# ShawnHymel/ei-keyword-spotting

Hardware: AMD Instinct MI355X
Metric: 1s@16kHz clips/sec (MFCC+CNN) (higher is better)
Workload: dtype f32

## Files before the change

ei-keyword-spotting_amd/csrc/kws_api.cpp:

```cpp
#include "kws_internal.h"

#pragma GCC visibility push(default)
extern "C" {

EI_IMPULSE_ERROR kws_create(const void *blob, size_t nbytes, int device, kws_handle **out)
{
    if (!blob || !out) return fail(KWS_ERROR_BAD_ARGUMENT, "null argument");
    *out = nullptr;
    kws_handle *h = new kws_handle();
    h->device = device;
    if (!parse_model(blob, nbytes, h->model)) { delete h; return fail(KWS_ERROR_BAD_ARGUMENT, "not a valid .kwsm model blob"); }
    int ndev = 0;
    if (hipGetDeviceCount(&ndev) != hipSuccess || ndev <= 0) {
        delete h;
        return fail(KWS_ERROR_HIP, "no HIP device available (libkws_mi355x has no CPU fallback)");
    }
    if (device < 0 || device >= ndev) { delete h; return fail(KWS_ERROR_HIP, "device %d out of range (%d devices)", device, ndev); }
    if (hipSetDevice(device) != hipSuccess) { delete h; return fail(KWS_ERROR_HIP, "hipSetDevice(%d) failed", device); }
    hipDeviceProp_t prop;
    if (hipGetDeviceProperties(&prop, device) == hipSuccess) h->n_cu = prop.multiProcessorCount;
    EI_IMPULSE_ERROR e = build_dsp_plan(h);
    if (e == EI_IMPULSE_OK) e = build_nn_plan(h);
    if (e == EI_IMPULSE_OK) e = build_fast_plans(h);
    if (e != EI_IMPULSE_OK) { kws_destroy(h); return e; }
// ... 13 lines not shown
    while ((n = fread(tmp, 1, sizeof(tmp), f)) > 0) buf.insert(buf.end(), tmp, tmp + n);
    fclose(f);
    return kws_create(buf.data(), buf.size(), device, out);
}

void kws_destroy(kws_handle *h)
{
    if (!h) return;
    kws_sdk_forget_default(h);
    (void)hipSetDevice(h->device);
    if (h->scratch_ev) { (void)hipEventSynchronize(h->scratch_ev); (void)hipEventDestroy(h->scratch_ev); }
    for (void *p : h->dev_allocs) (void)hipFree(p);
    if (h->s_mfcc) (void)hipFree(h->s_mfcc);
    if (h->s_q) (void)hipFree(h->s_q);
    if (h->d_flags) (void)hipFree(h->d_flags);
    if (h->d_flags2) (void)hipFree(h->d_flags2);
    if (h->d_flags3) (void)hipFree(h->d_flags3);
    if (h->s_cep) (void)hipFree(h->s_cep);
    if (h->scan_release) h->scan_release(h);
    for (hipEvent_t ev : h->gen_tune.ev) if (ev) (void)hipEventDestroy(ev);
    for (auto &g : h->g_sets) for (void *p : { (void *)g.ws, (void *)g.mfcc, (void *)g.feat }) if (p) (void)hipFree(p);
    for (int k = 0; k < 2; ++k) {
        for (void *p : { (void *)h->pipe.pcm[k], (void *)h->pipe.s[k], (void *)h->pipe.f[k], (void *)h->pipe.q[k] }) if (p) (void)hipFree(p);
        if (h->pipe.st[k]) (void)hipStreamDestroy(h->pipe.st[k]);
    }
    for (void *p : { (void *)h->ws.d_x, (void *)h->ws.d_f, (void *)h->ws.d_s, (void *)h->ws.d_w, (void *)h->ws.d_q })
        if (p) (void)hipFree(p);
    for (void *p : { (void *)h->ws.h_x, (void *)h->ws.h_s, (void *)h->ws.h_f })
        if (p) (void)hipHostFree(p);
    for (hipEvent_t ev : h->ws.ev) if (ev) (void)hipEventDestroy(ev);
// ... 123 lines not shown
    *count = 0;
    std::lock_guard<std::mutex> lk(h->mu);
    if (!h->d_flags2) return EI_IMPULSE_OK;
    HIP_TRY(hipSetDevice(h->device));
    HIP_TRY(hipDeviceSynchronize());
    int n = 0;
    HIP_TRY(hipMemcpy(&n, h->d_flags2, sizeof(int), hipMemcpyDeviceToHost));
    *count = (size_t)n;
    return EI_IMPULSE_OK;
}

static EI_IMPULSE_ERROR ensure_flags(kws_handle *h, size_t B)
{
    if (B + 1 <= h->flags_cap) return EI_IMPULSE_OK;
    if (h->d_flags) (void)hipFree(h->d_flags);
    if (h->d_flags2) (void)hipFree(h->d_flags2);
    if (h->d_flags3) (void)hipFree(h->d_flags3);
    h->d_flags = h->d_flags2 = h->d_flags3 = nullptr; h->flags_cap = 0;
    HIP_TRY(hipMalloc((void **)&h->d_flags, (B + 1) * sizeof(int)));
    HIP_TRY(hipMalloc((void **)&h->d_flags2, (B + 1) * sizeof(int)));
    HIP_TRY(hipMalloc((void **)&h->d_flags3, (B + 1) * sizeof(int)));
    HIP_TRY(hipMemset(h->d_flags2, 0, sizeof(int)));
    h->flags_cap = B + 1;
    return EI_IMPULSE_OK;
}

static EI_IMPULSE_ERROR classify_fast_device(kws_handle *h, const int16_t *pcm, size_t B, float *scores, float *fx, bool want_f, int8_t *q,
                                             hipStream_t s);
static EI_IMPULSE_ERROR classify_device(kws_handle *h, const int16_t *pcm, size_t B, float *scores, float *f, int8_t *q, hipStream_t s);
int grid_cap_mfcc(const kws_handle *h) { return h->n_cu * 8; }
int grid_cap_nn(const kws_handle *h) { return h->n_cu * 4; }

static const size_t kGenTuneMinClips = 2048;
static int generic_chunk_begin(kws_handle *h, size_t B, hipStream_t s, bool *mine)
{
    *mine = false;
    const char *fe = KWS_DEV_ENV("KWS_DEV_GENERIC_LCH");
// ... 414 lines not shown
    if (rc) return fail(KWS_ERROR_HIP, "quantise kernel launch failed: %s", hipGetErrorString((hipError_t)rc));
    return kws_nn_batch_device(h, h->s_q, B, scores, nullptr, nullptr, nullptr, stream);
}

static EI_IMPULSE_ERROR rerun_flagged_device(kws_handle *h, const int16_t *pcm, size_t B, float *scores, float *fx, bool want_f, int8_t *q, hipStream_t s)
{
    static const bool skip = KWS_DEV_ENV("KWS_DEV_FAST_NO_RERUN") != nullptr;
    if (skip) return EI_IMPULSE_OK;
    const size_t F = h->model.nn_input_frame_size;
    if (B > h->cep_cap) {
        if (h->s_cep) (void)hipFree(h->s_cep);
        h->s_cep = nullptr; h->cep_cap = 0;
        HIP_TRY(hipMalloc((void **)&h->s_cep, B * F * sizeof(float)));
        h->cep_cap = B;
    }
    HIP_TRY(hipMemsetAsync(h->d_flags2, 0, sizeof(int), s));
    int rc = kws_launch_spectral(h->dsp, pcm, 0, (int)B, h->s_cep, nullptr, 0, grid_cap_mfcc(h), s, h->d_flags);
    if (rc) return fail(KWS_ERROR_HIP, "MFCC kernel launch failed: %s", hipGetErrorString((hipError_t)rc));
    const bool fused = scores && h->is_float && h->fast_fused_ok;
    if (!scores || (fused && want_f) || !fused) {
        rc = kws_launch_fast_from_cepstra(h->dsp, h->fast_plain, h->d_fast_plain, h->s_cep, (int)B, nullptr, (h->is_float || want_f) ? fx : nullptr, q,
                                          h->nn.in_scale, h->nn.in_zp, h->d_flags2, h->d_flags2 + 1, h->n_cu, s, h->d_flags);
        if (rc) return fail(KWS_ERROR_HIP, "fast kernel launch failed: %s", hipGetErrorString((hipError_t)rc));
        if (fused) HIP_TRY(hipMemsetAsync(h->d_flags3, 0, sizeof(int), s));
    }
    if (fused) {
        int *const fl = want_f ? h->d_flags3 : h->d_flags2;
        rc = kws_launch_fast_from_cepstra(h->dsp, h->fast_fused_cep, h->d_fast_fused_cep, h->s_cep, (int)B, scores, nullptr, nullptr, h->nn.in_scale, h->nn.in_zp,
                                          fl, fl + 1, h->n_cu, s, h->d_flags, h->tap_logits);
        if (rc) return fail(KWS_ERROR_HIP, "fast kernel launch failed: %s", hipGetErrorString((hipError_t)rc));
    } else if (scores) {
// ... 7 lines not shown
    if (rc) return fail(KWS_ERROR_HIP, "CMVN kernel launch failed: %s", hipGetErrorString((hipError_t)rc));
    if (!scores) return EI_IMPULSE_OK;
    if (h->is_float) rc = kws_launch_nn_f32(h->nnf, h->d_nnf, fx, (int)B, scores, h->tap_logits, h->n_cu, s, h->d_flags2);
    else if (!ran_nn) rc = kws_launch_nn(h->nn, q, (int)B, scores, nullptr, h->pooled_tap_bytes, nullptr, nullptr, grid_cap_nn(h), s, h->d_flags2);
    if (rc) return fail(KWS_ERROR_HIP, "NN kernel launch failed: %s", hipGetErrorString((hipError_t)rc));
    return EI_IMPULSE_OK;
}

static EI_IMPULSE_ERROR classify_fast_device(kws_handle *h, const int16_t *pcm, size_t B, float *scores, float *fx, bool want_f, int8_t *q,
                                             hipStream_t s)
{
    if (B > 0x7fffffff) return fail(KWS_ERROR_BAD_ARGUMENT, "batch too large");
    if (((uintptr_t)pcm & 15) != 0) return fail(KWS_ERROR_BAD_ARGUMENT, "pcm must be 16-byte aligned");
    EI_IMPULSE_ERROR e = ensure_flags(h, B);
    if (e) return e;
    HIP_TRY(hipMemsetAsync(h->d_flags, 0, sizeof(int), s));
    const bool fused = scores && h->is_float && h->fast_fused_ok;
    int rc = 0;
    if (h->model.dsp.block == DSP_BLOCK_MFE) {
        const KwsDspPlan &P = h->dsp;
        const int rows = P.n_frames, cols = P.n_filters;
        if (rows > (cols > 16 ? 51 : 52) || P.win_size < (cols > 16 ? 17 : 13))
            return fail(KWS_ERROR_UNSUPPORTED_MODEL, "%d frames x %d filters, window %d outside the MFE normalisation kernel's limits", rows, cols, P.win_size);
        rc = kws_launch_fast(P, h->fast_plain, h->d_fast_plain, pcm, (int)B, nullptr, fx, nullptr, h->nn.in_scale, h->nn.in_zp, h->d_flags, h->d_flags + 1, h->n_cu, s);
        if (rc) return fail(KWS_ERROR_HIP, "fast kernel launch failed: %s (is the gfx950 code object present?)", hipGetErrorString((hipError_t)rc));
        rc = kws_launch_mfe_norm(fx, (int)B, rows, cols, P.win_size, P.pad_map, rows + 2 * P.pad, grid_cap_nn(h), s);
        if (!rc && q) rc = kws_launch_quantize(fx, q, B * h->model.nn_input_frame_size, h->nn.in_scale, h->nn.in_zp, s);
        if (rc) return fail(KWS_ERROR_HIP, "MFE block launch failed: %s", hipGetErrorString((hipError_t)rc));
        if (!scores) return EI_IMPULSE_OK;
        if (h->is_float) return nn_f32_device(h, fx, B, scores, h->tap_logits, s);
        rc = kws_launch_nn(h->nn, q, (int)B, scores, nullptr, h->pooled_tap_bytes, nullptr, nullptr, grid_cap_nn(h), s);
        if (rc) return fail(KWS_ERROR_HIP, "NN kernel launch failed: %s", hipGetErrorString((hipError_t)rc));
        return EI_IMPULSE_OK;
// ... 14 lines not shown
        if (h->fast_entry_tier >= 3) {
            HIP_TRY(hipMemsetAsync(h->d_flags2, 0, sizeof(int), s));
            if (!scores) return mfcc_fused_device(h, pcm, 0, B, fx, q, s);
            return classify_device(h, pcm, B, scores, fx, q, s);
        }
        const size_t F = h->model.nn_input_frame_size;
        if (B > h->cep_cap) {
            if (h->s_cep) (void)hipFree(h->s_cep);
            h->s_cep = nullptr; h->cep_cap = 0;
            HIP_TRY(hipMalloc((void **)&h->s_cep, B * F * sizeof(float)));
            h->cep_cap = B;
        }
        if ((e = spectral_device(h, h->dsp, pcm, 0, B, h->s_cep, nullptr, s))) return e;
        return cmvn_nn_fast_device(h, h->s_cep, B, scores, s, 0, 0, want_f ? fx : nullptr, q);
    }
    if (scores && !h->is_float && h->fast_q_ok) {
        rc = kws_launch_fast(h->dsp, h->fast_q, h->d_fast_q, pcm, (int)B, scores, want_f ? fx : nullptr, q != h->s_q ? q : nullptr, h->nn.in_scale, h->nn.in_zp,
                             h->d_flags, h->d_flags + 1, h->n_cu, s, h->d_nn);
        if (rc) return fail(KWS_ERROR_HIP, "fast kernel launch failed: %s (is the gfx950 code object present?)", hipGetErrorString((hipError_t)rc));
        return rerun_flagged_device(h, pcm, B, scores, fx, want_f, q, s);
    }
#ifdef KWS_DEV_SWITCHES
    if (fused && KWS_DEV_ENV("KWS_DEV_FAST_SPLIT")) {
        rc = kws_launch_fast(h->dsp, h->fast_plain, h->d_fast_plain, pcm, (int)B, nullptr, fx, nullptr, h->nn.in_scale, h->nn.in_zp, h->d_flags, h->d_flags + 1, h->n_cu, s);
        if (rc) return fail(KWS_ERROR_HIP, "fast kernel launch failed: %s", hipGetErrorString((hipError_t)rc));
        HIP_TRY(hipMemsetAsync(h->d_flags3, 0, sizeof(int), s));
        rc = kws_launch_fast_from_cepstra(h->dsp, h->fast_fused_cep, h->d_fast_fused_cep, fx, (int)B, scores, nullptr, nullptr, h->nn.in_scale, h->nn.in_zp,
                                          h->d_flags3, h->d_flags3 + 1, h->n_cu, s, nullptr, h->tap_logits, 1);
        if (rc) return fail(KWS_ERROR_HIP, "fast kernel launch failed: %s", hipGetErrorString((hipError_t)rc));
        return EI_IMPULSE_OK;
    }
#endif
    if (fused && want_f) {
        rc = kws_launch_fast(h->dsp, h->fast_plain, h->d_fast_plain, pcm, (int)B, nullptr, fx, nullptr, h->nn.in_scale, h->nn.in_zp, h->d_flags, h->d_flags + 1,
                             h->n_cu, s);
        if (rc) return fail(KWS_ERROR_HIP, "fast kernel launch failed: %s (is the gfx950 code object present?)", hipGetErrorString((hipError_t)rc));
        HIP_TRY(hipMemsetAsync(h->d_flags3, 0, sizeof(int), s));
    }
    const KwsFastPlan &FP = fused ? h->fast_fused : h->fast_plain;
    int *const fl = (fused && want_f) ? h->d_flags3 : h->d_flags;
    rc = kws_launch_fast(h->dsp, FP, fused ? h->d_fast_fused : h->d_fast_plain, pcm, (int)B, scores, fused ? nullptr : fx, fused ? nullptr : q, h->nn.in_scale,
                         h->nn.in_zp, fl, fl + 1, h->n_cu, s, nullptr, h->tap_logits);
    if (rc) return fail(KWS_ERROR_HIP, "fast kernel launch failed: %s (is the gfx950 code object present?)", hipGetErrorString((hipError_t)rc));
    if (scores && !fused) {
        if (h->is_float) { if ((e = nn_f32_device(h, fx, B, scores, h->tap_logits, s))) return e; }
        else {
            rc = kws_launch_nn(h->nn, q, (int)B, scores, nullptr, h->pooled_tap_bytes, nullptr, nullptr, grid_cap_nn(h), s);
            if (rc) return fail(KWS_ERROR_HIP, "NN kernel launch failed: %s", hipGetErrorString((hipError_t)rc));
        }
    }
    return rerun_flagged_device(h, pcm, B, scores, fx, want_f, q, s);
}

static EI_IMPULSE_ERROR classify_device(kws_handle *h, const int16_t *pcm, size_t B, float *scores, float *f, int8_t *q, hipStream_t s)
{
    EI_IMPULSE_ERROR e;
    if (h->is_float) {
        e = mfcc_fused_device(h, pcm, 0, B, f, nullptr, s);
// ... 139 lines not shown
```

ei-keyword-spotting_amd/csrc/kws_fast.h:

```cpp
#pragma once
#include <stdint.h>

#include "kws_plan.h"

#define KWS_FAST_MAX_BLOCKS 8
#define KWS_FAST_NZ_MAX 12
#define KWS_FAST_NZ2 8
#define KWS_FAST_DCT_GROUPS 5
#define KWS_FAST_MEL_CHUNK 8
#define KWS_FAST_CMVN_EXT 8
#define KWS_FAST_XS 144
#define KWS_FAST_WAVE 64
#ifndef KWS_FAST_WPS
#define KWS_FAST_WPS 2
#endif
#define KWS_FAST_ZF 320

struct KwsFastBlock {
    int in_w, in_c, in_cp;
    int out_c, taps, pad_left, out_w;
    int pool, pool_stride, pool_w;
    int in_stride;
    int m_tiles, n_tiles;
    int vrows;
// ... 43 lines not shown
    int fs, f_floats, r1_floats, wave_floats, shared_floats, n_waves;
    int zero_off;
    int sink_off;
    int stash_off;
    const float *shared_init;
    int qnet, q_floats;
    int mfe;
    int fuse, n_blocks;
    KwsFastBlock blk[KWS_FAST_MAX_BLOCKS];
    int fc_in, fc_out, fc_w_off, fc_b_off;
    float fc_min, fc_max, beta;
    int n_labels;
    int wps;
    int twl_off;
    int *tickets;
};
```

ei-keyword-spotting_amd/csrc/kws_fast.hip:

```cpp
#include <atomic>

#include "kws_device.h"
#include "kws_fast.h"
#if KWS_FAST_WPS >= 3
#define kws_fast_kernel kws_fast_kernel_w3
#define kws_launch_fast kws_launch_fast_w3
#define kws_launch_fast_prof kws_launch_fast_prof_w3
#endif
#include "kws_nn_int8_dev.h"

typedef float v4f __attribute__((ext_vector_type(4)));
#if KWS_FAST_WPS >= 3
#define KWS_OPAQUE3(v) asm volatile("" : "+v"(v))
#define KWS_FAST_SINK (shared + FP.sink_off)
#else
#define KWS_OPAQUE3(v) do { } while (0)
#define KWS_FAST_SINK (F + FP.sink_off)
#endif
static_assert(KWS_FAST_ZF == KWS_ZF && KWS_FAST_WAVE == KWS_WAVE, "kws_fast.h mirrors kws_device.h");

template <int CTRL> __device__ __forceinline__ float dpp_mov(float v)
{
    return __int_as_float(__builtin_amdgcn_update_dpp(0, __float_as_int(v), CTRL, 0xf, 0xf, true));
}
// ... 770 lines not shown
    }
    WAVE_SYNC();
    return vacc;
}

#define KWS_FAST_NPHASE 20
#define FPH(i) do { if (PROF) { const long long now_ = clock64(); ph[i] += now_ - tlast; tlast = now_; } } while (0)

template <int NZ, int DG, bool PROF = false, bool FROM_CEP = false, bool NET = true, int QCP = 0, bool MFE = false>
__global__ __launch_bounds__(256 * KWS_FAST_WPS, KWS_FAST_WPS) void kws_fast_kernel(KwsDspPlan P, const KwsFastPlan *__restrict__ FPp, const int16_t *__restrict__ pcm, int n_clips,
                                                          float *__restrict__ scores, float *__restrict__ features,
                                                          int8_t *__restrict__ q_out, float in_scale, int in_zp,
                                                          int *__restrict__ flag_count, int *__restrict__ flag_list,
                                                          long long *__restrict__ prof_out = nullptr, const float *__restrict__ cep = nullptr,
                                                          const KwsNnPlan *__restrict__ QNp = nullptr, const int *__restrict__ sel = nullptr,
                                                          float *__restrict__ tap_logits = nullptr, int feat_in = 0)
{
    static_assert(QCP == 0 || !NET, "the int8 network follows the feature-emitting form");
    static_assert(!MFE || (!NET && QCP == 0 && !FROM_CEP && !PROF), "the MFE form is the spectral prefix: mel energies to HBM");
    const KwsFastPlan &FP = *FPp;
    extern __shared__ __attribute__((aligned(16))) float lds[];
    const int lane = threadIdx.x & (KWS_WAVE - 1), wave = __builtin_amdgcn_readfirstlane((int)(threadIdx.x >> 6));
    if (FROM_CEP && (int)blockIdx.x * (int)(blockDim.x >> 6) >= sel_count(sel, n_clips)) return;
    float *shared = lds;
    float *F = lds + FP.shared_floats + FP.q_floats + wave * FP.wave_floats;
    float *R1 = F + FP.f_floats;
    float *xw = R1, *pw = R1;
    for (int i = threadIdx.x; i < FP.shared_floats; i += blockDim.x) shared[i] = FP.shared_init[i];
    for (int i = lane; i < FP.r1_floats; i += KWS_WAVE) R1[i] = 0.0f;
    constexpr int Q_HEAD = 48 * 256, Q_WB1 = Q_HEAD + ((KWS_HEAD_BYTES + 15) & ~15), Q_WB2 = Q_WB1 + (QCP == 16 ? 4 : 16) * KWS_WAVE * 16,
                  Q_RQ = Q_WB2 + 4 * KWS_WAVE * 16;
    if constexpr (QCP != 0) {
        unsigned char *const qs = (unsigned char *)(lds + FP.shared_floats);
        const KwsNnPlan &QN = *QNp;
        for (int i = threadIdx.x * 4; i < QN.blk[0].out_c * 256; i += blockDim.x * 4) *(int *)(qs + i) = *(const int *)(QN.blk[0].add_lut + i);
        for (int i = threadIdx.x * 4; i < QN.blk[1].out_c * 256; i += blockDim.x * 4) *(int *)(qs + 32 * 256 + i) = *(const int *)(QN.blk[1].add_lut + i);
// ... 397 lines not shown
                    prow[0] = pdc;
                }
                esum = half_wave_sum(esum);
                if (t == 0 && live_t) *((pair_tail && half == 1) ? stash + 47 : elog + ft) = fast_log(esum == 0.0f ? FLT_EPSILON : esum);
            }
            mel_phase(KWS_FAST_MEL_CHUNK * n_pass, pair_tail ? 2 : n_tail, 1, pair_tail ? (int)(stash - img) - nfr * fs : 0);
            have_stash = pair_tail;
            WAVE_SYNC();
        }

        if constexpr (!MFE) {
            int lane_l = lane;
            asm volatile("" : "+v"(lane_l));
            const int lm = lane_l & 15, lq = lane_l >> 4;
            float dB[DG][2][2];
#pragma unroll
            for (int g = 0; g < DG; ++g)
#pragma unroll
                for (int i = 0; i < 2; ++i)
#pragma unroll
                    for (int nt = 0; nt < 2; ++nt) dB[g][i][nt] = dct_frag[((g * 2 + i) * 2 + nt) * KWS_WAVE + lane_l];
            const float *arow = img + lm * fs + 2 * lq;
            float e0 = 0.0f;
            if (lane_l < nfr) e0 = elog[lane_l];
            v4f acc[4][2];
            __builtin_amdgcn_s_setprio(1);
#pragma unroll
            for (int rnd = 0; rnd < 2; ++rnd) {
                float2 a[2][DG];
#pragma unroll
                for (int m2 = 0; m2 < 2; ++m2)
#pragma unroll
                    for (int g = 0; g < DG; ++g) a[m2][g] = *(const float2 *)(arow + 16 * (2 * rnd + m2) * fs + 8 * g);
#pragma unroll
                for (int m2 = 0; m2 < 2; ++m2) { acc[2 * rnd + m2][0] = v4f{ 0.f, 0.f, 0.f, 0.f }; acc[2 * rnd + m2][1] = v4f{ 0.f, 0.f, 0.f, 0.f }; }
#pragma unroll
// ... 260 lines not shown
    if (lane == 0) {
        const int gone = __hip_atomic_fetch_add(FP.tickets + 1, 1, __ATOMIC_RELAXED, __HIP_MEMORY_SCOPE_AGENT);
        if (gone == (int)(gridDim.x * (blockDim.x >> 6)) - 1) {
            __hip_atomic_store(FP.tickets, 0, __ATOMIC_RELAXED, __HIP_MEMORY_SCOPE_AGENT);
            __hip_atomic_store(FP.tickets + 1, 0, __ATOMIC_RELAXED, __HIP_MEMORY_SCOPE_AGENT);
        }
    }
#endif
    if (PROF && blockIdx.x == 0 && threadIdx.x == 0 && prof_out)
        for (int i = 0; i < KWS_FAST_NPHASE; ++i) prof_out[i] = ph[i];
}

#ifndef KWS_FAST_NO_LAUNCHERS
#if KWS_FAST_WPS < 3
int kws_launch_fast_w3(const KwsDspPlan &P, const KwsFastPlan &FP, const KwsFastPlan *d_plan, const int16_t *pcm, int n_clips, float *scores, float *features,
                       int8_t *q_out, float in_scale, int in_zp, int *flag_count, int *flag_list, int n_cu, hipStream_t stream, const KwsNnPlan *d_nn, float *tap_logits);
int kws_launch_fast_prof_w3(const KwsDspPlan &P, const KwsFastPlan &FP, const KwsFastPlan *d_plan, const int16_t *pcm, int n_clips, float *scores,
                            int *flag_count, int *flag_list, int n_cu, long long *prof_out, hipStream_t stream);
#endif
template <int NZ, int DG, bool PROF, bool FROM_CEP = false, bool NET = true, int QCP = 0, bool MFE = false>
static int launch_fast_t(const KwsDspPlan &P, const KwsFastPlan &FP, const KwsFastPlan *d_plan, const int16_t *pcm, int n_clips, float *scores,
                         float *features, int8_t *q_out, float in_scale, int in_zp, int *flag_count, int *flag_list, int n_cu,
                         long long *prof_out, hipStream_t stream, const float *cep = nullptr, const KwsNnPlan *d_nn = nullptr, const int *sel = nullptr,
                         float *tap_logits = nullptr, int feat_in = 0)
{
    const size_t smem = ((size_t)FP.shared_floats + FP.q_floats + (size_t)FP.n_waves * FP.wave_floats) * sizeof(float);
    static std::atomic<unsigned long long> attr_done{ 0 };
    int dev = 0;
    if (hipGetDevice(&dev) != hipSuccess) return (int)hipGetLastError();
    const unsigned long long bit = 1ull << (dev & 63);
    if (!(attr_done.load(std::memory_order_acquire) & bit)) {
        if (hipFuncSetAttribute((const void *)kws_fast_kernel<NZ, DG, PROF, FROM_CEP, NET, QCP, MFE>, hipFuncAttributeMaxDynamicSharedMemorySize, 160 * 1024) != hipSuccess)
            return (int)hipGetLastError();
        attr_done.fetch_or(bit, std::memory_order_release);
    }
    const int per_wg = FP.n_waves;
    int grid = (n_clips + per_wg - 1) / per_wg;
    if (grid > n_cu) grid = n_cu;
#if KWS_FAST_WPS >= 3
    if (!FP.tickets) return (int)hipErrorInvalidValue;
#endif
    hipLaunchKernelGGL((kws_fast_kernel<NZ, DG, PROF, FROM_CEP, NET, QCP, MFE>), dim3(grid), dim3(KWS_WAVE * FP.n_waves), smem, stream, P, d_plan, pcm, n_clips, scores,
                       features, q_out, in_scale, in_zp, flag_count, flag_list, prof_out, cep, d_nn, sel, tap_logits, feat_in);
    return (int)hipGetLastError();
}

int kws_launch_fast(const KwsDspPlan &P, const KwsFastPlan &FP, const KwsFastPlan *d_plan, const int16_t *pcm, int n_clips, float *scores,
                    float *features, int8_t *q_out, float in_scale, int in_zp, int *flag_count, int *flag_list, int n_cu, hipStream_t stream,
                    const KwsNnPlan *d_nn, float *tap_logits)
{
    (void)hipGetLastError();
    if (n_clips <= 0) return 0;
#define KWS_FAST_ARGS P, FP, d_plan, pcm, n_clips, scores, features, q_out, in_scale, in_zp, flag_count, flag_list, n_cu, nullptr, stream
#define KWS_FAST_NARGS KWS_FAST_ARGS, nullptr, nullptr, nullptr, tap_logits
#if KWS_FAST_WPS >= 3
    if (FP.wps != KWS_FAST_WPS || FP.qnet || FP.mfe || !FP.fuse) return (int)hipErrorInvalidValue;
#define KWS_FAST_PLAIN(...) ((int)hipErrorInvalidValue)
#else
#define KWS_FAST_PLAIN(...) (__VA_ARGS__)
    if (FP.wps >= 3) return kws_launch_fast_w3(P, FP, d_plan, pcm, n_clips, scores, features, q_out, in_scale, in_zp, flag_count, flag_list, n_cu, stream, d_nn, tap_logits);
    if (FP.qnet) {
#define KWS_FAST_QARGS P, FP, d_plan, pcm, n_clips, scores, features, q_out, in_scale, in_zp, flag_count, flag_list, n_cu, nullptr, stream, nullptr, d_nn
        if (FP.qnet == 16 && FP.dct_groups == 4)
            return FP.nz <= 4 ? launch_fast_t<4, 4, false, false, false, 16>(KWS_FAST_QARGS) : FP.nz <= 8 ? launch_fast_t<8, 4, false, false, false, 16>(KWS_FAST_QARGS)
                                                                                                          : launch_fast_t<KWS_FAST_NZ_MAX, 4, false, false, false, 16>(KWS_FAST_QARGS);
        if (FP.qnet == 64 && FP.dct_groups == 5)
            return FP.nz <= 4 ? launch_fast_t<4, 5, false, false, false, 64>(KWS_FAST_QARGS) : FP.nz <= 8 ? launch_fast_t<8, 5, false, false, false, 64>(KWS_FAST_QARGS)
                                                                                                          : launch_fast_t<KWS_FAST_NZ_MAX, 5, false, false, false, 64>(KWS_FAST_QARGS);
        return (int)hipErrorInvalidValue;
    }
    if (FP.mfe) {
        if (scores || q_out || !features) return (int)hipErrorInvalidValue;
        if (FP.dct_groups == 4)
            return FP.nz <= 4 ? launch_fast_t<4, 4, false, false, false, 0, true>(KWS_FAST_ARGS) : FP.nz <= 8 ? launch_fast_t<8, 4, false, false, false, 0, true>(KWS_FAST_ARGS)
                                                                                                            : launch_fast_t<KWS_FAST_NZ_MAX, 4, false, false, false, 0, true>(KWS_FAST_ARGS);
        if (FP.dct_groups == 5)
            return FP.nz <= 4 ? launch_fast_t<4, 5, false, false, false, 0, true>(KWS_FAST_ARGS) : FP.nz <= 8 ? launch_fast_t<8, 5, false, false, false, 0, true>(KWS_FAST_ARGS)
// ... 58 lines not shown
```

ei-keyword-spotting_amd/csrc/kws_fast_plan.cpp:

```cpp
#include "kws_internal.h"
#include <atomic>
#include <cstdlib>

static const int kLdsBytes = 160 * 1024;

static int round_up(int v, int m) { return (v + m - 1) / m * m; }

static uint16_t f32_to_f16(float f)
{
    uint32_t u;
    memcpy(&u, &f, sizeof u);
    const uint32_t sign = (u >> 16) & 0x8000u;
    u &= 0x7fffffffu;
    if (u >= 0x47800000u) return (uint16_t)(sign | (u > 0x7f800000u ? 0x7e00u : 0x7c00u));
    if (u < 0x38800000u) {
        if (u < 0x33000000u) return (uint16_t)sign;
        const int shift = 126 - (int)(u >> 23);
        const uint32_t m = (u & 0x7fffffu) | 0x800000u;
        uint32_t h = m >> shift;
        const uint32_t rem = m & ((1u << shift) - 1u), half = 1u << (shift - 1);
        if (rem > half || (rem == half && (h & 1u))) h++;
        return (uint16_t)(sign | h);
    }
    uint32_t h = ((u - 0x38000000u) >> 13);
// ... 140 lines not shown
        F.c0_abs = scale * kFloorCep * per_dev;
        F.c0_rel = scale * std::min(kappa, kappa_0) * per_dev;
        F.c0_inv_rows = 1.0f / (float)nfr;
    }
    F.sys_t2 = (h->is_float && h->gain.calibrated) ? kSysRatio * kSysRatio : 0.0f;
    F.pad_off = (int)shared.size();
    for (int v : pmap) { float f; memcpy(&f, &v, sizeof f); shared.push_back(f); }
    F.sil_off = -1;
    if ((int)h->fast_sil_row.size() == ncep && !KWS_DEV_ENV("KWS_DEV_FAST_NO_SILENT_ROW")) {
        while (shared.size() & 3) shared.push_back(0.0f);
        F.sil_off = (int)shared.size();
        for (int c = 0; c < 32; c++) shared.push_back((c >= 1 && c <= NF / 2 && c < ncep) ? h->fast_sil_row[(size_t)c] : 0.0f);
    }
}

static EI_IMPULSE_ERROR build_fast_dsp(kws_handle *h, KwsFastPlan &F, std::vector<float> &shared)
{
    const Model &m = h->model;
    const DspCfg &c = m.dsp;
    const KwsDspPlan &P = h->dsp;
    const int NF = c.num_filters, nfr = P.n_frames, ncep = P.n_cepstral;
    F.mfe = c.block == DSP_BLOCK_MFE ? 1 : 0;
    if (P.generic) return fail(KWS_ERROR_UNSUPPORTED_MODEL, "fast mode serves the configurations of the tuned MFCC kernel (fft 256, 32 / 40 filters, "
                                                            "up to 52 aligned frames); this model runs on the general kernels");
    if (c.fft_length != 256) return fail(KWS_ERROR_UNSUPPORTED_MODEL, "fast mode: fft_length %d (kernel is built for 256)", c.fft_length);
    if (NF != 32 && NF != 40) return fail(KWS_ERROR_UNSUPPORTED_MODEL, "fast mode: %d mel filters (the kernel is instantiated for 32 and 40)", NF);
    if ((ncep <= 16 || F.wps >= 3) && nfr <= 52) { F.cr = 13; F.cg = 16; }
    else if (nfr <= 51) { F.cr = 17; F.cg = 20; }
    else return fail(KWS_ERROR_UNSUPPORTED_MODEL, "fast mode: %d frames x %d cepstra outside the cmvnw layouts", nfr, ncep);
    if (nfr < 2) return fail(KWS_ERROR_UNSUPPORTED_MODEL, "fast mode: %d frames", nfr);

// ... 114 lines not shown
        h_twiddles(c.fft_length / 2, tw);
        h_super_twiddles(c.fft_length / 2, stw);
        while (shared.size() & 3) shared.push_back(0.0f);
        F.twl_off = (int)shared.size();
        for (int fl = 0; fl < 8; fl++)
            for (int a = 0; a < 4; a++)
                for (int m = 1; m <= 3; m++) { const float2 v = tw[(size_t)m * (fl + 8 * a)]; shared.push_back(v.x); shared.push_back(v.y); }
        for (int fl = 0; fl < 8; fl++)
            for (int q = 0; q < 8; q++) {
                const int k = fl + 8 * (q & 3) + 32 * (q >> 2);
                const float2 v = stw[(size_t)(k == 0 ? c.fft_length / 4 : k) - 1];
                shared.push_back(v.x); shared.push_back(v.y);
            }
    }
    while (shared.size() & 3) shared.push_back(0.0f);
    F.dct_off = (int)shared.size();
    shared.insert(shared.end(), frag.begin(), frag.end());
    return EI_IMPULSE_OK;
}

static void fast_wave_floats(const kws_handle *h, KwsFastPlan &F, int need_f, int need_r1)
{
    const int nfr = h->dsp.n_frames;
    if (F.wps >= 3) {
        F.f_floats = round_up(std::max(nfr * F.fs + nfr, need_f), 4) + 48;
    } else {
        F.f_floats = round_up(std::max(nfr * F.fs + nfr, need_f), 4) + KWS_FAST_WAVE + 48;
        F.sink_off = F.f_floats - KWS_FAST_WAVE - 48;
    }
    F.stash_off = F.f_floats - 48;
// ... 75 lines not shown
    std::vector<float> shared;
    EI_IMPULSE_ERROR e = build_fast_dsp(h, F, shared);
    if (e) return e;
    F.fs = h->dsp.n_filters + 4;
    F.fuse = 0;
    F.n_labels = (int)h->model.labels.size();
    F.qnet = qcp;
    F.q_floats = (int)((kws_fast_qnet_bytes(qcp) + 15) / 16 * 4);
    if (!h->d_nn) {
        std::vector<KwsNnPlan> one(1, h->nn);
        if ((e = h->upload(one, &h->d_nn))) return e;
    }
    return finish_fast_plan(h, F, shared, 24 * 8 + 96, 72 * qcp / 4);
}

static EI_IMPULSE_ERROR build_fast_fused(kws_handle *h, int wps, KwsFastPlan &F)
{
    memset(&F, 0, sizeof(F));
    F.wps = wps;
    if (!h->is_float) return fail(KWS_ERROR_UNSUPPORTED_MODEL, "fast mode: the fused network is float32 (int8 graphs keep their exact kernels)");
    if (h->fast_plain.mfe) return fail(KWS_ERROR_UNSUPPORTED_MODEL, "fast mode: the MFE block's normalisation sits between the front end and the network (not fused)");
    const KwsNnPlanF32 &N = h->nnf;
    if (N.n_blocks > KWS_FAST_MAX_BLOCKS) return fail(KWS_ERROR_UNSUPPORTED_MODEL, "fast mode: %d conv blocks", N.n_blocks);
    if (N.fc_out > KWS_FAST_WAVE) return fail(KWS_ERROR_UNSUPPORTED_MODEL, "fast mode: %d outputs", N.fc_out);
    std::vector<float> shared;
    EI_IMPULSE_ERROR e = build_fast_dsp(h, F, shared);
    if (e) return e;
    F.fuse = 1;
    F.n_blocks = N.n_blocks;
    F.n_labels = N.n_labels;
    F.fs = h->dsp.n_filters + 4;
    int need[2] = { 0, 0 };
    std::vector<uint16_t> hfrag[KWS_FAST_MAX_BLOCKS];
    const bool hconv_on = !KWS_DEV_ENV("KWS_DEV_FAST_F32_CONV");
    while (shared.size() & 3) shared.push_back(0.0f);
    F.zero_off = (int)shared.size();
    shared.resize(shared.size() + 64, 0.0f);
    for (int b = 0; b < N.n_blocks; b++) {
        const KwsConvBlockF32 &s = N.blk[b];
        KwsFastBlock &k = F.blk[b];
        k.dw = s.depthwise ? 1 : 0; k.mult = s.depth_mult;
        k.in_w = s.in_w; k.in_c = s.in_c; k.in_cp = round_up(s.in_c, 8);
        k.out_c = s.out_c; k.taps = s.taps; k.pad_left = s.pad_left; k.out_w = s.out_w;
        k.pool = s.pool; k.pool_stride = s.pool_stride; k.pool_w = s.pool_w;
        k.in_stride = b == 0 ? F.fs : k.in_cp + 4;
        k.m_tiles = (s.out_w + 15) / 16; k.n_tiles = (s.out_c + 15) / 16;
// ... 115 lines not shown
        k.dw_seg_rows = (k.out_w + k.dw_nseg - 1) / k.dw_nseg;
    }
    return finish_fast_plan(h, F, shared, need[0], need[1]);
}

EI_IMPULSE_ERROR build_fast_plans(kws_handle *h)
{
    if (h->is_float && !h->dsp.generic && h->nnf.n_blocks > 0 && h->nnf.blk[0].in_w == h->dsp.n_frames && h->nnf.blk[0].in_c == h->dsp.n_cepstral)
        kws_calibrate_gain(h);
    record_silent_row(h);
    h->fast_plain_ok = build_fast_plain(h) == EI_IMPULSE_OK;
    if (!h->fast_plain_ok) h->fast_why = kws_last_error();
    int want_wps = h->fast_entry_tier <= 1 ? 3 : 2, min_waves3 = 11;
    if (const char *ev = KWS_DEV_ENV("KWS_DEV_FAST_WPS")) { want_wps = atoi(ev) >= 3 ? 3 : 2; min_waves3 = 4; }
    h->fast_fused_ok = h->fast_plain_ok && build_fast_fused(h, want_wps, h->fast_fused) == EI_IMPULSE_OK;
    if (h->fast_plain_ok && want_wps >= 3 && (!h->fast_fused_ok || h->fast_fused.n_waves < min_waves3))
        h->fast_fused_ok = build_fast_fused(h, 2, h->fast_fused) == EI_IMPULSE_OK;
    if (h->fast_fused_ok) {
        if (h->fast_fused.wps >= 3) h->fast_fused_ok = build_fast_fused(h, 2, h->fast_fused_cep) == EI_IMPULSE_OK;
        else { h->fast_fused_cep = h->fast_fused; h->d_fast_fused_cep = h->d_fast_fused; }
    }
    if (h->fast_plain_ok && !h->fast_fused_ok) h->fast_why = kws_last_error();
    h->fast_q_ok = h->fast_plain_ok && !h->is_float && build_fast_q(h) == EI_IMPULSE_OK;
    if (h->fast_plain_ok && !h->is_float && !h->fast_q_ok) h->fast_why = kws_last_error();
    return EI_IMPULSE_OK;
}
```

ei-keyword-spotting_amd/csrc/kws_internal.h:

```cpp
#pragma once
#include <hip/hip_runtime.h>

#include <float.h>
#include <math.h>
#include <stdarg.h>
#include <stdio.h>
#include <stdlib.h>
#include <string.h>
#include <time.h>

#include <mutex>
#include <string>
#include <map>
#include <vector>

#include "../../include/kws/kws.h"
#include "kws_plan.h"
#include "kws_fast.h"

int kws_launch_spectral(const KwsDspPlan &P, const void *pcm, int pcm_is_float, int n_clips, float *mfcc_out, const float *wrap,
                        int out_stride, int grid_cap, hipStream_t stream, const int *sel = nullptr);
int kws_launch_maf(float *scores, float *running_sum, float *maf_buf, int n, int buf_idx, int taps, hipStream_t stream);
int kws_launch_unring(const float *src, float *dst, int n_streams, int rows, int cols, int ring_rows, int head, hipStream_t stream);
int kws_launch_mfe(const KwsDspPlan &P, const void *pcm, int pcm_is_float, int n_clips, float *mel_out, float *energy_out, const float *wrap,
// ... 5 lines not shown
                               int in_zp, int grid_cap, long long *prof_out, hipStream_t stream);
int kws_launch_cmvn_nn(const KwsDspPlan &P, const KwsNnPlan &N, const float *mfcc, int n_clips, float *features, int8_t *q_out,
                       float *scores, int8_t *tap_pooled, int pooled_stride, int8_t *tap_fc, int8_t *tap_out_q, int grid_cap,
                       int *ran_nn, hipStream_t stream, const int *sel = nullptr);
int kws_launch_fast_from_cepstra(const KwsDspPlan &P, const KwsFastPlan &FP, const KwsFastPlan *d_plan, const float *cep, int n_clips, float *scores,
                                 float *features, int8_t *q_out, float in_scale, int in_zp, int *flag_count, int *flag_list, int n_cu, hipStream_t stream,
                                 const int *sel = nullptr, float *tap_logits = nullptr, int feat_in = 0);
int kws_launch_nn_f32(const KwsNnPlanF32 &N, const KwsNnPlanF32 *d_plan, const float *features, int n_clips, float *scores,
                      float *tap_logits, int n_cu, hipStream_t stream, const int *sel = nullptr);
size_t kws_nn_f32_smem_bytes(const KwsNnPlanF32 &N, int n_waves);
void kws_nn_f32_pick_blocking(KwsConvBlockF32 *k);
int kws_launch_nn(const KwsNnPlan &N, const int8_t *q_in, int n_clips, float *scores, int8_t *tap_pooled,
                  int pooled_stride, int8_t *tap_fc, int8_t *tap_out_q, int grid_cap, hipStream_t stream, const int *sel = nullptr);
int kws_launch_fast(const KwsDspPlan &P, const KwsFastPlan &FP, const KwsFastPlan *d_plan, const int16_t *pcm, int n_clips, float *scores, float *features,
                    int8_t *q_out, float in_scale, int in_zp, int *flag_count, int *flag_list, int n_cu, hipStream_t stream, const KwsNnPlan *d_nn = nullptr,
                    float *tap_logits = nullptr);
size_t kws_fast_qnet_bytes(int qcp);
int kws_launch_fast_prof(const KwsDspPlan &P, const KwsFastPlan &FP, const KwsFastPlan *d_plan, const int16_t *pcm, int n_clips, float *scores,
                         int *flag_count, int *flag_list, int n_cu, long long *prof_out, hipStream_t stream);
int kws_launch_mix_audio(const float *words, const int *word_len, size_t word_stride, const float *noise, const int *start, float word_vol,
                         float bg_vol, int n, size_t n_clips, int16_t *out, hipStream_t stream);
int kws_launch_quantize(const float *f, int8_t *q, size_t n, float scale, int zp, hipStream_t stream);
int kws_launch_resample(const float *in, size_t n_in, float *out, size_t n_out, size_t n_valid, double ratio, const double *win, const double *delta, int nwin,
                        int precision, int exact, const double *treg, hipStream_t stream);
size_t kws_generic_ws_bytes(const KwsDspPlan &P, int grid);
bool kws_generic_uses_lds(const KwsDspPlan &P);
int kws_launch_spectral_generic(const KwsDspPlan &P, const void *pcm, int pcm_is_float, int n_clips, float *mfcc_out, const float *wrap,
                                int out_stride, float *ws, int grid, int lch , hipStream_t stream);
int kws_launch_cmvn_generic(const KwsDspPlan &P, const float *mfcc, int n_clips, float *features, int8_t *q_out, float in_scale, int in_zp,
                            hipStream_t stream);
int kws_launch_synth(uint32_t seed, uint32_t first_clip, uint32_t n_clips, uint32_t clip_len, int16_t *out, hipStream_t stream);
// ... 133 lines not shown
    struct Gain { std::vector<float> col; float sigma_net = 0.0f, total = 0.0f; int calibrated = 0, n_inputs = 0; } gain;
    KwsFastPlan fast_plain{}, fast_fused{}, fast_q{};
    const KwsFastPlan *d_fast_plain = nullptr, *d_fast_fused = nullptr, *d_fast_q = nullptr;
    KwsFastPlan fast_fused_cep{};
    const KwsFastPlan *d_fast_fused_cep = nullptr;
    const KwsNnPlan *d_nn = nullptr;
    bool fast_plain_ok = false, fast_fused_ok = false, fast_q_ok = false;
    std::string fast_why;
    std::vector<float> fast_guard_coef[2][4];
    int fast_dev_overrides = 0;
    int fast_entry_tier = 1;
    std::vector<float> fast_sil_row;
    std::vector<float> fast_gain_used;
    int mode = KWS_MODE_EXACT;
    int *d_flags = nullptr;
    int *d_flags2 = nullptr;
    int *d_flags3 = nullptr;
    float *tap_logits = nullptr;
    float *s_cep = nullptr;
    struct KwsScanScratch *scan = nullptr;
    void (*scan_release)(kws_handle *) = nullptr;
    size_t flags_cap = 0, cep_cap = 0;

    template <typename T> EI_IMPULSE_ERROR upload(const std::vector<T> &v, const T **out)
    {
        void *d = nullptr;
        size_t nb = std::max<size_t>(v.size() * sizeof(T), 16);
        HIP_TRY(hipMalloc(&d, nb));
        dev_allocs.push_back(d);
        if (!v.empty()) HIP_TRY(hipMemcpy(d, v.data(), v.size() * sizeof(T), hipMemcpyHostToDevice));
// ... 72 lines not shown
```

Before: 52.70 million.

## Zero flag counters inside fast kernel via double-buffered flags instead of memsets

Removes the per-call hipMemsetAsync launches for the flag counters. It double-buffers d_flags so the fast kernel's first thread clears the next call's counter and the rerun counter. It also adds an opt-in compact fused plan that keeps the DCT fragment in global memory instead of LDS, which can raise the wave count. The compact path is gated behind a dev env switch. The ping-pong scheme assumes the counter for the next call is consumed before the kernel that zeroes it runs.

```diff
diff --git a/ei-keyword-spotting_amd/csrc/kws_api.cpp b/ei-keyword-spotting_amd/csrc/kws_api.cpp
--- a/ei-keyword-spotting_amd/csrc/kws_api.cpp
+++ b/ei-keyword-spotting_amd/csrc/kws_api.cpp
@@ -51,6 +51,7 @@
     if (h->s_mfcc) (void)hipFree(h->s_mfcc);
     if (h->s_q) (void)hipFree(h->s_q);
     if (h->d_flags) (void)hipFree(h->d_flags);
+    if (h->d_flags_alt) (void)hipFree(h->d_flags_alt);
     if (h->d_flags2) (void)hipFree(h->d_flags2);
     if (h->d_flags3) (void)hipFree(h->d_flags3);
     if (h->s_cep) (void)hipFree(h->s_cep);
@@ -204,13 +205,16 @@
 {
     if (B + 1 <= h->flags_cap) return EI_IMPULSE_OK;
     if (h->d_flags) (void)hipFree(h->d_flags);
+    if (h->d_flags_alt) (void)hipFree(h->d_flags_alt);
     if (h->d_flags2) (void)hipFree(h->d_flags2);
     if (h->d_flags3) (void)hipFree(h->d_flags3);
-    h->d_flags = h->d_flags2 = h->d_flags3 = nullptr; h->flags_cap = 0;
+    h->d_flags = h->d_flags_alt = h->d_flags2 = h->d_flags3 = nullptr; h->flags_cap = 0;
     HIP_TRY(hipMalloc((void **)&h->d_flags, (B + 1) * sizeof(int)));
+    HIP_TRY(hipMalloc((void **)&h->d_flags_alt, (B + 1) * sizeof(int)));
     HIP_TRY(hipMalloc((void **)&h->d_flags2, (B + 1) * sizeof(int)));
     HIP_TRY(hipMalloc((void **)&h->d_flags3, (B + 1) * sizeof(int)));
     HIP_TRY(hipMemset(h->d_flags2, 0, sizeof(int)));
+    HIP_TRY(hipMemset(h->d_flags_alt, 0, sizeof(int)));
     h->flags_cap = B + 1;
     return EI_IMPULSE_OK;
 }
@@ -655,7 +659,6 @@
         HIP_TRY(hipMalloc((void **)&h->s_cep, B * F * sizeof(float)));
         h->cep_cap = B;
     }
-    HIP_TRY(hipMemsetAsync(h->d_flags2, 0, sizeof(int), s));
     int rc = kws_launch_spectral(h->dsp, pcm, 0, (int)B, h->s_cep, nullptr, 0, grid_cap_mfcc(h), s, h->d_flags);
     if (rc) return fail(KWS_ERROR_HIP, "MFCC kernel launch failed: %s", hipGetErrorString((hipError_t)rc));
     const bool fused = scores && h->is_float && h->fast_fused_ok;
@@ -693,9 +696,9 @@
     if (((uintptr_t)pcm & 15) != 0) return fail(KWS_ERROR_BAD_ARGUMENT, "pcm must be 16-byte aligned");
     EI_IMPULSE_ERROR e = ensure_flags(h, B);
     if (e) return e;
-    HIP_TRY(hipMemsetAsync(h->d_flags, 0, sizeof(int), s));
     const bool fused = scores && h->is_float && h->fast_fused_ok;
     int rc = 0;
+    if (h->model.dsp.block == DSP_BLOCK_MFE || (h->fast_entry_tier >= 2 && (scores || want_f || q))) HIP_TRY(hipMemsetAsync(h->d_flags, 0, sizeof(int), s));
     if (h->model.dsp.block == DSP_BLOCK_MFE) {
         const KwsDspPlan &P = h->dsp;
         const int rows = P.n_frames, cols = P.n_filters;
@@ -740,16 +743,20 @@
         if ((e = spectral_device(h, h->dsp, pcm, 0, B, h->s_cep, nullptr, s))) return e;
         return cmvn_nn_fast_device(h, h->s_cep, B, scores, s, 0, 0, want_f ? fx : nullptr, q);
     }
+    std::swap(h->d_flags, h->d_flags_alt);
+    int *const zero_a = h->d_flags_alt, *const zero_b = h->d_flags2;
+    auto first_launch_failed = [h]() { std::swap(h->d_flags, h->d_flags_alt); };
     if (scores && !h->is_float && h->fast_q_ok) {
         rc = kws_launch_fast(h->dsp, h->fast_q, h->d_fast_q, pcm, (int)B, scores, want_f ? fx : nullptr, q != h->s_q ? q : nullptr, h->nn.in_scale, h->nn.in_zp,
-                             h->d_flags, h->d_flags + 1, h->n_cu, s, h->d_nn);
-        if (rc) return fail(KWS_ERROR_HIP, "fast kernel launch failed: %s (is the gfx950 code object present?)", hipGetErrorString((hipError_t)rc));
+                             h->d_flags, h->d_flags + 1, h->n_cu, s, h->d_nn, nullptr, zero_a, zero_b);
+        if (rc) { first_launch_failed(); return fail(KWS_ERROR_HIP, "fast kernel launch failed: %s (is the gfx950 code object present?)", hipGetErrorString((hipError_t)rc)); }
         return rerun_flagged_device(h, pcm, B, scores, fx, want_f, q, s);
     }
 #ifdef KWS_DEV_SWITCHES
     if (fused && KWS_DEV_ENV("KWS_DEV_FAST_SPLIT")) {
-        rc = kws_launch_fast(h->dsp, h->fast_plain, h->d_fast_plain, pcm, (int)B, nullptr, fx, nullptr, h->nn.in_scale, h->nn.in_zp, h->d_flags, h->d_flags + 1, h->n_cu, s);
-        if (rc) return fail(KWS_ERROR_HIP, "fast kernel launch failed: %s", hipGetErrorString((hipError_t)rc));
+        rc = kws_launch_fast(h->dsp, h->fast_plain, h->d_fast_plain, pcm, (int)B, nullptr, fx, nullptr, h->nn.in_scale, h->nn.in_zp, h->d_flags, h->d_flags + 1, h->n_cu, s,
+                             nullptr, nullptr, zero_a, zero_b);
+        if (rc) { first_launch_failed(); return fail(KWS_ERROR_HIP, "fast kernel launch failed: %s", hipGetErrorString((hipError_t)rc)); }
         HIP_TRY(hipMemsetAsync(h->d_flags3, 0, sizeof(int), s));
         rc = kws_launch_fast_from_cepstra(h->dsp, h->fast_fused_cep, h->d_fast_fused_cep, fx, (int)B, scores, nullptr, nullptr, h->nn.in_scale, h->nn.in_zp,
                                           h->d_flags3, h->d_flags3 + 1, h->n_cu, s, nullptr, h->tap_logits, 1);
@@ -759,15 +766,19 @@
 #endif
     if (fused && want_f) {
         rc = kws_launch_fast(h->dsp, h->fast_plain, h->d_fast_plain, pcm, (int)B, nullptr, fx, nullptr, h->nn.in_scale, h->nn.in_zp, h->d_flags, h->d_flags + 1,
-                             h->n_cu, s);
-        if (rc) return fail(KWS_ERROR_HIP, "fast kernel launch failed: %s (is the gfx950 code object present?)", hipGetErrorString((hipError_t)rc));
+                             h->n_cu, s, nullptr, nullptr, zero_a, zero_b);
+        if (rc) { first_launch_failed(); return fail(KWS_ERROR_HIP, "fast kernel launch failed: %s (is the gfx950 code object present?)", hipGetErrorString((hipError_t)rc)); }
         HIP_TRY(hipMemsetAsync(h->d_flags3, 0, sizeof(int), s));
     }
+    const bool first = !(fused && want_f);
     const KwsFastPlan &FP = fused ? h->fast_fused : h->fast_plain;
     int *const fl = (fused && want_f) ? h->d_flags3 : h->d_flags;
     rc = kws_launch_fast(h->dsp, FP, fused ? h->d_fast_fused : h->d_fast_plain, pcm, (int)B, scores, fused ? nullptr : fx, fused ? nullptr : q, h->nn.in_scale,
-                         h->nn.in_zp, fl, fl + 1, h->n_cu, s, nullptr, h->tap_logits);
-    if (rc) return fail(KWS_ERROR_HIP, "fast kernel launch failed: %s (is the gfx950 code object present?)", hipGetErrorString((hipError_t)rc));
+                         h->nn.in_zp, fl, fl + 1, h->n_cu, s, nullptr, h->tap_logits, first ? zero_a : nullptr, first ? zero_b : nullptr);
+    if (rc) {
+        if (first) first_launch_failed();
+        return fail(KWS_ERROR_HIP, "fast kernel launch failed: %s (is the gfx950 code object present?)", hipGetErrorString((hipError_t)rc));
+    }
     if (scores && !fused) {
         if (h->is_float) { if ((e = nn_f32_device(h, fx, B, scores, h->tap_logits, s))) return e; }
         else {
diff --git a/ei-keyword-spotting_amd/csrc/kws_fast.h b/ei-keyword-spotting_amd/csrc/kws_fast.h
--- a/ei-keyword-spotting_amd/csrc/kws_fast.h
+++ b/ei-keyword-spotting_amd/csrc/kws_fast.h
@@ -81,4 +81,5 @@
     int wps;
     int twl_off;
     int *tickets;
+    const float *dct_global;
 };
diff --git a/ei-keyword-spotting_amd/csrc/kws_fast.hip b/ei-keyword-spotting_amd/csrc/kws_fast.hip
--- a/ei-keyword-spotting_amd/csrc/kws_fast.hip
+++ b/ei-keyword-spotting_amd/csrc/kws_fast.hip
@@ -808,12 +808,17 @@
                                                           int *__restrict__ flag_count, int *__restrict__ flag_list,
                                                           long long *__restrict__ prof_out = nullptr, const float *__restrict__ cep = nullptr,
                                                           const KwsNnPlan *__restrict__ QNp = nullptr, const int *__restrict__ sel = nullptr,
-                                                          float *__restrict__ tap_logits = nullptr, int feat_in = 0)
+                                                          float *__restrict__ tap_logits = nullptr, int feat_in = 0,
+                                                          int *__restrict__ zero_a = nullptr, int *__restrict__ zero_b = nullptr)
 {
     static_assert(QCP == 0 || !NET, "the int8 network follows the feature-emitting form");
     static_assert(!MFE || (!NET && QCP == 0 && !FROM_CEP && !PROF), "the MFE form is the spectral prefix: mel energies to HBM");
     const KwsFastPlan &FP = *FPp;
     extern __shared__ __attribute__((aligned(16))) float lds[];
+    if (blockIdx.x == 0 && threadIdx.x == 0) {
+        if (zero_a) *zero_a = 0;
+        if (zero_b) *zero_b = 0;
+    }
     const int lane = threadIdx.x & (KWS_WAVE - 1), wave = __builtin_amdgcn_readfirstlane((int)(threadIdx.x >> 6));
     if (FROM_CEP && (int)blockIdx.x * (int)(blockDim.x >> 6) >= sel_count(sel, n_clips)) return;
     float *shared = lds;
@@ -1241,12 +1246,25 @@
             asm volatile("" : "+v"(lane_l));
             const int lm = lane_l & 15, lq = lane_l >> 4;
             float dB[DG][2][2];
-#pragma unroll
-            for (int g = 0; g < DG; ++g)
-#pragma unroll
-                for (int i = 0; i < 2; ++i)
-#pragma unroll
-                    for (int nt = 0; nt < 2; ++nt) dB[g][i][nt] = dct_frag[((g * 2 + i) * 2 + nt) * KWS_WAVE + lane_l];
+#if KWS_FAST_WPS >= 3
+            if (FP.dct_global) {
+                const __attribute__((address_space(1))) float *const dg = (const __attribute__((address_space(1))) float *)FP.dct_global + lane_l;
+#pragma unroll
+                for (int g = 0; g < DG; ++g)
+#pragma unroll
+                    for (int i = 0; i < 2; ++i)
+#pragma unroll
+                        for (int nt = 0; nt < 2; ++nt) dB[g][i][nt] = dg[((g * 2 + i) * 2 + nt) * KWS_WAVE];
+            } else
+#endif
+            {
+#pragma unroll
+                for (int g = 0; g < DG; ++g)
+#pragma unroll
+                    for (int i = 0; i < 2; ++i)
+#pragma unroll
+                        for (int nt = 0; nt < 2; ++nt) dB[g][i][nt] = dct_frag[((g * 2 + i) * 2 + nt) * KWS_WAVE + lane_l];
+            }
             const float *arow = img + lm * fs + 2 * lq;
             float e0 = 0.0f;
             if (lane_l < nfr) e0 = elog[lane_l];
@@ -1537,7 +1555,8 @@
 #ifndef KWS_FAST_NO_LAUNCHERS
 #if KWS_FAST_WPS < 3
 int kws_launch_fast_w3(const KwsDspPlan &P, const KwsFastPlan &FP, const KwsFastPlan *d_plan, const int16_t *pcm, int n_clips, float *scores, float *features,
-                       int8_t *q_out, float in_scale, int in_zp, int *flag_count, int *flag_list, int n_cu, hipStream_t stream, const KwsNnPlan *d_nn, float *tap_logits);
+                       int8_t *q_out, float in_scale, int in_zp, int *flag_count, int *flag_list, int n_cu, hipStream_t stream, const KwsNnPlan *d_nn, float *tap_logits,
+                       int *zero_a, int *zero_b);
 int kws_launch_fast_prof_w3(const KwsDspPlan &P, const KwsFastPlan &FP, const KwsFastPlan *d_plan, const int16_t *pcm, int n_clips, float *scores,
                             int *flag_count, int *flag_list, int n_cu, long long *prof_out, hipStream_t stream);
 #endif
@@ -1545,7 +1564,7 @@
 static int launch_fast_t(const KwsDspPlan &P, const KwsFastPlan &FP, const KwsFastPlan *d_plan, const int16_t *pcm, int n_clips, float *scores,
                          float *features, int8_t *q_out, float in_scale, int in_zp, int *flag_count, int *flag_list, int n_cu,
                          long long *prof_out, hipStream_t stream, const float *cep = nullptr, const KwsNnPlan *d_nn = nullptr, const int *sel = nullptr,
-                         float *tap_logits = nullptr, int feat_in = 0)
+                         float *tap_logits = nullptr, int feat_in = 0, int *zero_a = nullptr, int *zero_b = nullptr)
 {
     const size_t smem = ((size_t)FP.shared_floats + FP.q_floats + (size_t)FP.n_waves * FP.wave_floats) * sizeof(float);
     static std::atomic<unsigned long long> attr_done{ 0 };
@@ -1564,26 +1583,28 @@
     if (!FP.tickets) return (int)hipErrorInvalidValue;
 #endif
     hipLaunchKernelGGL((kws_fast_kernel<NZ, DG, PROF, FROM_CEP, NET, QCP, MFE>), dim3(grid), dim3(KWS_WAVE * FP.n_waves), smem, stream, P, d_plan, pcm, n_clips, scores,
-                       features, q_out, in_scale, in_zp, flag_count, flag_list, prof_out, cep, d_nn, sel, tap_logits, feat_in);
+                       features, q_out, in_scale, in_zp, flag_count, flag_list, prof_out, cep, d_nn, sel, tap_logits, feat_in, zero_a, zero_b);
     return (int)hipGetLastError();
 }
 
 int kws_launch_fast(const KwsDspPlan &P, const KwsFastPlan &FP, const KwsFastPlan *d_plan, const int16_t *pcm, int n_clips, float *scores,
                     float *features, int8_t *q_out, float in_scale, int in_zp, int *flag_count, int *flag_list, int n_cu, hipStream_t stream,
-                    const KwsNnPlan *d_nn, float *tap_logits)
+                    const KwsNnPlan *d_nn, float *tap_logits, int *zero_a, int *zero_b)
 {
     (void)hipGetLastError();
     if (n_clips <= 0) return 0;
-#define KWS_FAST_ARGS P, FP, d_plan, pcm, n_clips, scores, features, q_out, in_scale, in_zp, flag_count, flag_list, n_cu, nullptr, stream
-#define KWS_FAST_NARGS KWS_FAST_ARGS, nullptr, nullptr, nullptr, tap_logits
+#define KWS_FAST_ARGS0 P, FP, d_plan, pcm, n_clips, scores, features, q_out, in_scale, in_zp, flag_count, flag_list, n_cu, nullptr, stream
+#define KWS_FAST_ARGS KWS_FAST_ARGS0, nullptr, nullptr, nullptr, nullptr, 0, zero_a, zero_b
+#define KWS_FAST_NARGS KWS_FAST_ARGS0, nullptr, nullptr, nullptr, tap_logits, 0, zero_a, zero_b
 #if KWS_FAST_WPS >= 3
     if (FP.wps != KWS_FAST_WPS || FP.qnet || FP.mfe || !FP.fuse) return (int)hipErrorInvalidValue;
 #define KWS_FAST_PLAIN(...) ((int)hipErrorInvalidValue)
 #else
 #define KWS_FAST_PLAIN(...) (__VA_ARGS__)
-    if (FP.wps >= 3) return kws_launch_fast_w3(P, FP, d_plan, pcm, n_clips, scores, features, q_out, in_scale, in_zp, flag_count, flag_list, n_cu, stream, d_nn, tap_logits);
+    if (FP.wps >= 3)
+        return kws_launch_fast_w3(P, FP, d_plan, pcm, n_clips, scores, features, q_out, in_scale, in_zp, flag_count, flag_list, n_cu, stream, d_nn, tap_logits, zero_a, zero_b);
     if (FP.qnet) {
-#define KWS_FAST_QARGS P, FP, d_plan, pcm, n_clips, scores, features, q_out, in_scale, in_zp, flag_count, flag_list, n_cu, nullptr, stream, nullptr, d_nn
+#define KWS_FAST_QARGS KWS_FAST_ARGS0, nullptr, d_nn, nullptr, nullptr, 0, zero_a, zero_b
         if (FP.qnet == 16 && FP.dct_groups == 4)
             return FP.nz <= 4 ? launch_fast_t<4, 4, false, false, false, 16>(KWS_FAST_QARGS) : FP.nz <= 8 ? launch_fast_t<8, 4, false, false, false, 16>(KWS_FAST_QARGS)
                                                                                                           : launch_fast_t<KWS_FAST_NZ_MAX, 4, false, false, false, 16>(KWS_FAST_QARGS);
diff --git a/ei-keyword-spotting_amd/csrc/kws_fast_plan.cpp b/ei-keyword-spotting_amd/csrc/kws_fast_plan.cpp
--- a/ei-keyword-spotting_amd/csrc/kws_fast_plan.cpp
+++ b/ei-keyword-spotting_amd/csrc/kws_fast_plan.cpp
@@ -178,7 +178,7 @@
     }
 }
 
-static EI_IMPULSE_ERROR build_fast_dsp(kws_handle *h, KwsFastPlan &F, std::vector<float> &shared)
+static EI_IMPULSE_ERROR build_fast_dsp(kws_handle *h, KwsFastPlan &F, std::vector<float> &shared, bool dct_in_l2 = false)
 {
     const Model &m = h->model;
     const DspCfg &c = m.dsp;
@@ -323,6 +323,14 @@
             }
     }
     while (shared.size() & 3) shared.push_back(0.0f);
+    F.dct_global = nullptr;
+    if (dct_in_l2) {
+        F.dct_off = -1;
+        const float *dev = nullptr;
+        if ((e = h->upload(frag, &dev))) return e;
+        F.dct_global = dev;
+        return EI_IMPULSE_OK;
+    }
     F.dct_off = (int)shared.size();
     shared.insert(shared.end(), frag.begin(), frag.end());
     return EI_IMPULSE_OK;
@@ -428,7 +436,7 @@
     return finish_fast_plan(h, F, shared, 24 * 8 + 96, 72 * qcp / 4);
 }
 
-static EI_IMPULSE_ERROR build_fast_fused(kws_handle *h, int wps, KwsFastPlan &F)
+static EI_IMPULSE_ERROR build_fast_fused(kws_handle *h, int wps, KwsFastPlan &F, bool compact = false)
 {
     memset(&F, 0, sizeof(F));
     F.wps = wps;
@@ -438,12 +446,12 @@
     if (N.n_blocks > KWS_FAST_MAX_BLOCKS) return fail(KWS_ERROR_UNSUPPORTED_MODEL, "fast mode: %d conv blocks", N.n_blocks);
     if (N.fc_out > KWS_FAST_WAVE) return fail(KWS_ERROR_UNSUPPORTED_MODEL, "fast mode: %d outputs", N.fc_out);
     std::vector<float> shared;
-    EI_IMPULSE_ERROR e = build_fast_dsp(h, F, shared);
+    EI_IMPULSE_ERROR e = build_fast_dsp(h, F, shared, compact && wps >= 3);
     if (e) return e;
     F.fuse = 1;
     F.n_blocks = N.n_blocks;
     F.n_labels = N.n_labels;
-    F.fs = h->dsp.n_filters + 4;
+    F.fs = h->dsp.n_filters + (compact && wps >= 3 ? 0 : 4);
     int need[2] = { 0, 0 };
     std::vector<uint16_t> hfrag[KWS_FAST_MAX_BLOCKS];
     const bool hconv_on = !KWS_DEV_ENV("KWS_DEV_FAST_F32_CONV");
@@ -589,6 +597,11 @@
     int want_wps = h->fast_entry_tier <= 1 ? 3 : 2, min_waves3 = 11;
     if (const char *ev = KWS_DEV_ENV("KWS_DEV_FAST_WPS")) { want_wps = atoi(ev) >= 3 ? 3 : 2; min_waves3 = 4; }
     h->fast_fused_ok = h->fast_plain_ok && build_fast_fused(h, want_wps, h->fast_fused) == EI_IMPULSE_OK;
+    if (h->fast_fused_ok && h->fast_fused.wps >= 3 && h->fast_fused.n_waves < 12 && KWS_DEV_ENV("KWS_DEV_FAST_COMPACT")) {
+        const int padded_waves = h->fast_fused.n_waves;
+        if (build_fast_fused(h, want_wps, h->fast_fused, true) != EI_IMPULSE_OK || h->fast_fused.n_waves <= padded_waves)
+            h->fast_fused_ok = build_fast_fused(h, want_wps, h->fast_fused) == EI_IMPULSE_OK;
+    }
     if (h->fast_plain_ok && want_wps >= 3 && (!h->fast_fused_ok || h->fast_fused.n_waves < min_waves3))
         h->fast_fused_ok = build_fast_fused(h, 2, h->fast_fused) == EI_IMPULSE_OK;
     if (h->fast_fused_ok) {
diff --git a/ei-keyword-spotting_amd/csrc/kws_internal.h b/ei-keyword-spotting_amd/csrc/kws_internal.h
--- a/ei-keyword-spotting_amd/csrc/kws_internal.h
+++ b/ei-keyword-spotting_amd/csrc/kws_internal.h
@@ -43,7 +43,7 @@
                   int pooled_stride, int8_t *tap_fc, int8_t *tap_out_q, int grid_cap, hipStream_t stream, const int *sel = nullptr);
 int kws_launch_fast(const KwsDspPlan &P, const KwsFastPlan &FP, const KwsFastPlan *d_plan, const int16_t *pcm, int n_clips, float *scores, float *features,
                     int8_t *q_out, float in_scale, int in_zp, int *flag_count, int *flag_list, int n_cu, hipStream_t stream, const KwsNnPlan *d_nn = nullptr,
-                    float *tap_logits = nullptr);
+                    float *tap_logits = nullptr, int *zero_a = nullptr, int *zero_b = nullptr);
 size_t kws_fast_qnet_bytes(int qcp);
 int kws_launch_fast_prof(const KwsDspPlan &P, const KwsFastPlan &FP, const KwsFastPlan *d_plan, const int16_t *pcm, int n_clips, float *scores,
                          int *flag_count, int *flag_list, int n_cu, long long *prof_out, hipStream_t stream);
@@ -207,6 +207,7 @@
     std::vector<float> fast_gain_used;
     int mode = KWS_MODE_EXACT;
     int *d_flags = nullptr;
+    int *d_flags_alt = nullptr;
     int *d_flags2 = nullptr;
     int *d_flags3 = nullptr;
     float *tap_logits = nullptr;
```

After: 52.88 million, median of 6. No clear change (+0.3%).
